# kubegems/modelx

Measured on AMD Instinct MI355X. Metric: push+pull GiB/s end-to-end (S3->HBM, digest-verified), 1/2/4/8 MI355X, higher is better.
Workload: dtype uint8; 1 GPU; model=synthetic-8GiB-blob, global_batch=1, seq_len=0, parallelism=dp1-presigned-s3-pipelined

## Files before the change

core/src/engine.cpp:

```cpp
#include <hip/hip_runtime.h>
#include <openssl/evp.h>
#include <pybind11/pybind11.h>
#include <pybind11/stl.h>

#include <atomic>
#include <chrono>
#include <condition_variable>
#include <cstring>
#include <deque>
#include <map>
#include <memory>
#include <mutex>
#include <queue>
#include <stdexcept>
#include <string_view>
#include <thread>
#include <unordered_set>
#include <vector>

#include "modelx/device_abi.hpp"
#include "modelx/http.hpp"
#include "modelx/tar_host.hpp"
#include "modelx/zstd_core.hpp"
#include "modelx/zstd_host.hpp"

namespace py = pybind11;
using namespace modelx;
using modelx::abi::ChunkLeavesDesc;
using modelx::abi::CopySeg;
using modelx::abi::kDedupMaxProbes;
using modelx::abi::PackSeg;
using modelx::abi::TarEntry;
using zstdhost::SeekEntry;

static uint32_t zstd_flags() {
  static uint32_t f = [] {
    const char* v = getenv("MODELX_ZSTD_FLAGS");
    return v ? (uint32_t)atoi(v) : 0u;
  }();
  return f;
}

#define HIP_CHECK(expr)                                                                 \
  do {                                                                                  \
    hipError_t _e = (expr);                                                             \
    if (_e != hipSuccess)                                                               \
      throw std::runtime_error(std::string("HIP error: ") + hipGetErrorString(_e) +     \
                               " at " #expr);                                           \
  } while (0)

namespace {

double now_s() {
  return std::chrono::duration<double>(std::chrono::steady_clock::now().time_since_epoch())
      .count();
}

uint64_t expected_leaf_count(uint64_t size, uint64_t chunk_size) {
  return size ? (size - 1) / chunk_size + 1 : 1;
}

uint32_t checked_leaf_count(const char* who, size_t leaves_bytes, uint64_t chunk_size,
                            uint64_t size) {
  if (chunk_size == 0) throw std::runtime_error(std::string(who) + ": chunk_size is 0");
  if (leaves_bytes % 32)
    throw std::runtime_error(std::string(who) + ": leaves length " +
                             std::to_string(leaves_bytes) + " is not a multiple of 32");
  uint64_t want = expected_leaf_count(size, chunk_size);
  if (leaves_bytes / 32 != want || want > UINT32_MAX)
    throw std::runtime_error(std::string(who) + ": " + std::to_string(leaves_bytes / 32) +
                             " leaves for " + std::to_string(size) + " bytes at chunk size " +
                             std::to_string(chunk_size) + " (expected " +
                             std::to_string(want) + ")");
  return static_cast<uint32_t>(want);
}

struct Slot {
  char* host = nullptr;
  hipEvent_t event = nullptr;
  size_t bytes = 0;
};

struct Range {
  uint64_t offset;
  uint64_t length;
};

class DeviceBuffer {
 public:
  DeviceBuffer() = default;
  explicit DeviceBuffer(size_t bytes) { HIP_CHECK(hipMalloc(&p_, bytes)); }
  DeviceBuffer(DeviceBuffer&& o) noexcept : p_(o.p_) { o.p_ = nullptr; }
  DeviceBuffer& operator=(DeviceBuffer&& o) noexcept {
    std::swap(p_, o.p_);
    return *this;
  }
  ~DeviceBuffer() {
    if (p_) hipFree(p_);
  }
  template <class T = void>
  T* get() const { return static_cast<T*>(p_); }
  explicit operator bool() const { return p_ != nullptr; }

 private:
  void* p_ = nullptr;
};

class DeviceScratch {
 public:
  template <class T = void>
  T* reserve(size_t bytes) {
    if (cap_ < bytes) {
      cap_ = 0;
      buf_ = DeviceBuffer();
      buf_ = DeviceBuffer(bytes);
      cap_ = bytes;
    }
    return buf_.get<T>();
  }

 private:
  DeviceBuffer buf_;
  size_t cap_ = 0;
};

class ConnPool {
 public:
  std::unique_ptr<http::ClientConn> checkout(const std::string& host, int port, bool tls) {
    std::lock_guard<std::mutex> lk(mu_);
    auto& v = pool_[(tls ? "https:" : "http:") + host + ":" + std::to_string(port)];
    if (!v.empty()) {
      auto c = std::move(v.back());
      v.pop_back();
      return c;
    }
    return std::make_unique<http::ClientConn>(host, port, tls);
  }
  void checkin(std::unique_ptr<http::ClientConn> c) {
    if (!c || !c->connected()) return;
    std::lock_guard<std::mutex> lk(mu_);
    auto& v = pool_[(c->tls() ? "https:" : "http:") + c->host() + ":" +
                    std::to_string(c->port())];
    if (v.size() < 64) v.push_back(std::move(c));
  }

 private:
  std::mutex mu_;
  std::map<std::string, std::vector<std::unique_ptr<http::ClientConn>>> pool_;
};

class GpuEngine {
 public:
  GpuEngine(int device, int num_slots, size_t slot_bytes, int num_streams)
      : device_(device), slot_bytes_(slot_bytes) {
    HIP_CHECK(hipSetDevice(device_));
    slots_.resize(num_slots);
    for (auto& s : slots_) {
      HIP_CHECK(hipHostMalloc(reinterpret_cast<void**>(&s.host), slot_bytes,
                              hipHostMallocDefault));
      HIP_CHECK(hipEventCreateWithFlags(&s.event, hipEventDisableTiming));
      free_.push(&s);
    }
    streams_.resize(num_streams);
    for (auto& st : streams_) HIP_CHECK(hipStreamCreateWithFlags(&st, hipStreamNonBlocking));
    HIP_CHECK(hipStreamCreateWithFlags(&hash_stream_, hipStreamNonBlocking));
    HIP_CHECK(hipEventCreateWithFlags(&zs_staged_, hipEventDisableTiming));
  }

  ~GpuEngine() {
    for (auto& st : streams_) hipStreamDestroy(st);
    hipStreamDestroy(hash_stream_);
    hipEventDestroy(zs_staged_);
    for (auto& s : slots_) {
      if (s.event) hipEventDestroy(s.event);
      if (s.host) hipHostFree(s.host);
    }
  }


  py::dict pull_to_device(const std::string& url,
                          const std::map<std::string, std::string>& headers, uint64_t size,
                          uintptr_t dst_ptr, int num_conns, uint64_t base_offset = 0) {
    std::string leaves;
    return pull_impl(url, headers, size, dst_ptr, num_conns, base_offset, 0, &leaves, nullptr);
  }

  py::dict pull_ranges_to_device(const std::string& url,
                                 const std::map<std::string, std::string>& headers,
                                 const std::vector<std::pair<uint64_t, uint64_t>>& ranges,
                                 uintptr_t dst_ptr, int num_conns) {
    std::string leaves;
    std::vector<Range> rs;
    uint64_t total = 0;
    for (auto& r : ranges) {
      for (uint64_t off = 0; off < r.second; off += slot_bytes_)
        rs.push_back({r.first + off, std::min<uint64_t>(slot_bytes_, r.second - off)});
      total += r.second;
    }
    return pull_impl(url, headers, total, dst_ptr, num_conns, 0, 0, &leaves, &rs);
  }

  py::tuple pull_to_device_hashed(const std::string& url,
                                  const std::map<std::string, std::string>& headers,
                                  uint64_t size, uintptr_t dst_ptr, int num_conns,
                                  uint64_t chunk_size) {
    std::string leaves;
    py::dict stats =
        pull_impl(url, headers, size, dst_ptr, num_conns, 0, chunk_size, &leaves, nullptr);
    return py::make_tuple(stats, py::bytes(leaves));
  }

  py::dict pull_impl(const std::string& url, const std::map<std::string, std::string>& headers,
                     uint64_t size, uintptr_t dst_ptr, int num_conns, uint64_t base_offset,
                     uint64_t hash_chunk, std::string* leaves_out,
                     const std::vector<Range>* explicit_ranges) {
    DeviceBuffer dleaves;
    uint32_t total_chunks = 0;
    if (hash_chunk) {
      if (slot_bytes_ % hash_chunk != 0)
        throw std::runtime_error("slot_bytes must be a multiple of chunk_size");
      total_chunks = size ? static_cast<uint32_t>((size + hash_chunk - 1) / hash_chunk) : 1;
      dleaves = DeviceBuffer(static_cast<size_t>(total_chunks) * 32);
    }
    py::gil_scoped_release release;
    HIP_CHECK(hipSetDevice(device_));
    double t0 = now_s();

    constexpr uint64_t kSlotsPerRequest = 4;
    std::vector<Range> ranges;
    if (explicit_ranges) {
      ranges = *explicit_ranges;
    } else {
      uint64_t super = slot_bytes_ * kSlotsPerRequest;
      for (uint64_t off = 0; off < size; off += super)
        ranges.push_back({off, std::min<uint64_t>(super, size - off)});
    }
    std::atomic<size_t> next_range{0};
    std::mutex err_mu;
    std::string error;
    std::atomic<uint64_t> net_bytes{0};
    std::atomic<long> net_ns{0};

    std::atomic<bool> done_submitting{false};
    std::thread reclaimer([&] {
      while (true) {
        Slot* s = nullptr;
        {
          std::unique_lock<std::mutex> lk(mu_);
          cv_pending_.wait(lk, [&] {
            return !pending_.empty() || (done_submitting.load() && pending_.empty());
          });
          if (pending_.empty()) break;
          s = pending_.front();
          pending_.pop_front();
        }
        hipEventSynchronize(s->event);
        {
          std::lock_guard<std::mutex> lk(mu_);
          free_.push(s);
        }
        cv_free_.notify_all();
      }
    });

    http::Url u = http::Url::parse(url);
    std::vector<std::thread> workers;
    std::atomic<int> stream_rr{0};
    for (int w = 0; w < num_conns; w++) {
      workers.emplace_back([&, w] {
        if (hipError_t e = hipSetDevice(device_); e != hipSuccess) {
          std::lock_guard<std::mutex> lk(err_mu);
          if (error.empty()) error = std::string("hip: ") + hipGetErrorString(e);
          return;
        }
        auto conn_holder = conn_pool_.checkout(u.host, u.port, u.scheme == "https");
        http::ClientConn& conn = *conn_holder;
        http::Headers h;
        for (auto& kv : headers) h[kv.first] = kv.second;
        while (true) {
          Range r;
          {
            size_t i = next_range.fetch_add(1);
            if (i >= ranges.size()) break;
            {
              std::lock_guard<std::mutex> lk(err_mu);
              if (!error.empty()) break;
            }
            r = ranges[i];
          }
          bool ok = false;
          for (int attempt = 0; attempt < 3 && !ok; attempt++) {
            double tn = now_s();
            if (!begin_range_fetch(conn, u, h, {r.offset + base_offset, r.length})) continue;
            ok = true;
            for (uint64_t poff = 0; poff < r.length && ok; poff += slot_bytes_) {
              uint64_t plen = std::min<uint64_t>(slot_bytes_, r.length - poff);
              Slot* slot = acquire_slot();
              if (!conn.read_body_exact(slot->host, plen)) {
                conn.close_fd();
                release_slot(slot);
                ok = false;
                break;
              }
              uint64_t abs_off = r.offset + poff;
              hipStream_t st = streams_[stream_rr.fetch_add(1) % streams_.size()];
              hipError_t e = hipMemcpyAsync(reinterpret_cast<char*>(dst_ptr) + abs_off,
                                            slot->host, plen, hipMemcpyHostToDevice, st);
              if (e == hipSuccess && hash_chunk) {
                uint32_t first_chunk = static_cast<uint32_t>(abs_off / hash_chunk);
                uint32_t n_chunks =
                    static_cast<uint32_t>((plen + hash_chunk - 1) / hash_chunk);
                e = modelx_sha256_chunk_leaves(
                    reinterpret_cast<char*>(dst_ptr) + abs_off, plen, hash_chunk,
                    dleaves.get<char>() + static_cast<size_t>(first_chunk) * 32,
                    n_chunks, st);
              }
              if (e == hipSuccess) e = hipEventRecord(slot->event, st);
              if (e != hipSuccess) {
                {
                  std::lock_guard<std::mutex> lk(err_mu);
                  if (error.empty()) error = std::string("hip: ") + hipGetErrorString(e);
                }
                release_slot(slot);
                ok = false;
                attempt = 3;
                break;
              }
              {
                std::lock_guard<std::mutex> lk(mu_);
                pending_.push_back(slot);
              }
              cv_pending_.notify_all();
            }
            if (ok) {
              net_ns.fetch_add(static_cast<long>((now_s() - tn) * 1e9));
              net_bytes.fetch_add(r.length);
            }
          }
          if (!ok) {
            std::lock_guard<std::mutex> lk(err_mu);
            if (error.empty()) error = "range fetch failed @" + std::to_string(r.offset);
            break;
          }
        }
        conn_pool_.checkin(std::move(conn_holder));
      });
    }
    for (auto& t : workers) t.join();
    done_submitting.store(true);
    cv_pending_.notify_all();
    reclaimer.join();
    for (auto& st : streams_) HIP_CHECK(hipStreamSynchronize(st));
    if (hash_chunk) {
      leaves_out->resize(static_cast<size_t>(total_chunks) * 32);
      HIP_CHECK(hipMemcpy(&(*leaves_out)[0], dleaves.get(), leaves_out->size(),
                          hipMemcpyDeviceToHost));
      dleaves = DeviceBuffer();
    }
    double t1 = now_s();
    {
      std::lock_guard<std::mutex> lk(err_mu);
      if (!error.empty()) throw std::runtime_error("pull_to_device: " + error);
    }
    py::gil_scoped_acquire acquire;
    py::dict stats;
    stats["seconds"] = t1 - t0;
    stats["bytes"] = size;
    stats["gib_per_s"] = size / (t1 - t0) / (1 << 30);
    stats["net_conn_seconds"] = net_ns.load() / 1e9;
    return stats;
  }


  py::bytes sha256_chunk_leaves(uintptr_t dev_ptr, uint64_t size, uint64_t chunk_size) {
    if (chunk_size == 0) throw std::runtime_error("sha256_chunk_leaves: chunk_size is 0");
    HIP_CHECK(hipSetDevice(device_));
    uint32_t nchunks = static_cast<uint32_t>(expected_leaf_count(size, chunk_size));
    std::string out;
    {
      py::gil_scoped_release release;
      DeviceBuffer dleaves(static_cast<size_t>(nchunks) * 32);
      HIP_CHECK(modelx_sha256_chunk_leaves(reinterpret_cast<void*>(dev_ptr), size, chunk_size,
                                           dleaves.get(), nchunks, hash_stream_));
      out.resize(static_cast<size_t>(nchunks) * 32);
      HIP_CHECK(hipStreamSynchronize(hash_stream_));
      HIP_CHECK(hipMemcpy(&out[0], dleaves.get(), out.size(), hipMemcpyDeviceToHost));
    }
    return py::bytes(out);
  }

  py::bytes sha256_multibuf(const std::vector<std::pair<uintptr_t, uint64_t>>& bufs) {
    HIP_CHECK(hipSetDevice(device_));
    uint32_t n = static_cast<uint32_t>(bufs.size());
    if (n == 0) return py::bytes("");
    std::vector<const void*> hptrs(n);
    std::vector<uint64_t> hlens(n);
    for (uint32_t i = 0; i < n; i++) {
      hptrs[i] = reinterpret_cast<const void*>(bufs[i].first);
      hlens[i] = bufs[i].second;
    }
    std::string out;
    {
      py::gil_scoped_release release;
      DeviceBuffer dptrs(n * sizeof(void*));
      DeviceBuffer dlens(n * sizeof(uint64_t));
      DeviceBuffer ddig(static_cast<size_t>(n) * 32);
      HIP_CHECK(hipMemcpyAsync(dptrs.get(), hptrs.data(), n * sizeof(void*),
                               hipMemcpyHostToDevice, hash_stream_));
      HIP_CHECK(hipMemcpyAsync(dlens.get(), hlens.data(), n * sizeof(uint64_t),
                               hipMemcpyHostToDevice, hash_stream_));
      HIP_CHECK(modelx_sha256_multibuf(dptrs.get<const void*>(), dlens.get<uint64_t>(), n,
                                       ddig.get(), hash_stream_));
      out.resize(static_cast<size_t>(n) * 32);
      HIP_CHECK(hipStreamSynchronize(hash_stream_));
      HIP_CHECK(hipMemcpy(&out[0], ddig.get(), out.size(), hipMemcpyDeviceToHost));
    }
    return py::bytes(out);
  }

  py::bytes read_device(uintptr_t src_ptr, uint64_t size) {
    HIP_CHECK(hipSetDevice(device_));
    std::string out(size, '\0');
    {
      py::gil_scoped_release release;
      HIP_CHECK(hipMemcpy(&out[0], reinterpret_cast<void*>(src_ptr), size,
                          hipMemcpyDeviceToHost));
    }
    return py::bytes(out);
  }

  py::bytes sha256_canonical_device(uintptr_t src_ptr, uint64_t size) {
    HIP_CHECK(hipSetDevice(device_));
    unsigned char md[32];
    {
      py::gil_scoped_release release;
      std::unique_ptr<EVP_MD_CTX, decltype(&EVP_MD_CTX_free)> ctx(EVP_MD_CTX_new(),
                                                                  &EVP_MD_CTX_free);
      if (!ctx || EVP_DigestInit_ex(ctx.get(), EVP_sha256(), nullptr) != 1)
        throw std::runtime_error("EVP sha256 init failed");
      hipError_t e = drain_device(src_ptr, size, [&](const char* p, uint64_t len) {
        EVP_DigestUpdate(ctx.get(), p, len);
        return true;
      });
      if (e != hipSuccess)
        throw std::runtime_error(std::string("sha256_canonical_device: hip: ") +
                                 hipGetErrorString(e));
      unsigned int mdlen = 0;
      EVP_DigestFinal_ex(ctx.get(), md, &mdlen);
    }
    return py::bytes(reinterpret_cast<char*>(md), 32);
  }


  py::dict push_part_from_device(const std::string& url, const std::string& method,
                                 const std::map<std::string, std::string>& headers,
                                 uintptr_t src_ptr, uint64_t size) {
    py::gil_scoped_release release;
    HIP_CHECK(hipSetDevice(device_));
    double t0 = now_s();
    http::Url u = http::Url::parse(url);
    auto conn_holder = conn_pool_.checkout(u.host, u.port, u.scheme == "https");
    http::ClientConn& conn = *conn_holder;
    http::Headers h;
    for (auto& kv : headers) h[kv.first] = kv.second;
    if (!conn.send_request(method, u.target(), h, static_cast<int64_t>(size)))
      throw std::runtime_error("push: send_request failed");
    bool sent = true;
    HIP_CHECK(drain_device(src_ptr, size, [&](const char* p, uint64_t len) {
      return sent = conn.send_body(p, len);
    }));
    if (!sent) throw std::runtime_error("push: send_body failed");
    int status = 0;
    http::Headers rh;
    if (!conn.read_response_head(&status, &rh)) throw std::runtime_error("push: no response");
    char drain[4096];
    while (conn.read_body(drain, sizeof drain) > 0) {
    }
    conn_pool_.checkin(std::move(conn_holder));
    double t1 = now_s();
    if (status < 200 || status >= 300)
      throw std::runtime_error("push: HTTP " + std::to_string(status));
    py::gil_scoped_acquire acquire;
    py::dict stats;
    stats["seconds"] = t1 - t0;
    stats["bytes"] = size;
    stats["status"] = status;
    return stats;
  }


  py::list tar_index(uintptr_t tar_ptr, uint64_t tar_len) {
    HIP_CHECK(hipSetDevice(device_));
    uint32_t max_entries = tarhost::kMaxIndexEntries;
    std::vector<TarEntry> entries;
    uint32_t count = 0, error = 0;
    {
      py::gil_scoped_release release;
      DeviceBuffer dentries(max_entries * sizeof(TarEntry));
      DeviceBuffer dcount_buf(2 * sizeof(uint32_t));
      uint32_t* dcount = dcount_buf.get<uint32_t>();
      HIP_CHECK(modelx_tar_index(reinterpret_cast<void*>(tar_ptr), tar_len,
                                 dentries.get<TarEntry>(), max_entries, dcount, dcount + 1,
                                 hash_stream_));
      HIP_CHECK(hipStreamSynchronize(hash_stream_));
      HIP_CHECK(hipMemcpy(&count, dcount, sizeof count, hipMemcpyDeviceToHost));
      HIP_CHECK(hipMemcpy(&error, dcount + 1, sizeof error, hipMemcpyDeviceToHost));
// ... 341 lines not shown
                    reinterpret_cast<uint8_t*>(dleaves + off[i] * 32), size, cs,
                    (uint32_t)off[i], 0};
      }
      ChunkLeavesDesc* ddescs = zs_descs_.reserve<ChunkLeavesDesc>(n * sizeof(ChunkLeavesDesc));
      HIP_CHECK(hipMemcpyAsync(ddescs, descs.data(), n * sizeof(ChunkLeavesDesc),
                               hipMemcpyHostToDevice, hash_stream_));
      HIP_CHECK(modelx_sha256_chunk_leaves_many(ddescs, (uint32_t)n, (uint32_t)total,
                                                hash_stream_));
      HIP_CHECK(hipStreamSynchronize(hash_stream_));
      host.resize(total * 32);
      HIP_CHECK(hipMemcpy(&host[0], dleaves, host.size(), hipMemcpyDeviceToHost));
    }
    for (size_t i = 0; i < n; i++)
      res.emplace_back(host.data() + off[i] * 32, (size_t)nchunks[i] * 32);
    return res;
  }

  static uint64_t zstd_compress_bound(uint64_t size, uint32_t frame_raw) {
    using namespace modelx::zstd;
    if (frame_raw == 0) frame_raw = 128 << 10;
    uint64_t nframes = size ? (size + frame_raw - 1) / frame_raw : 1;
    uint64_t stride = (uint64_t)frame_raw + 64 + 3 * ((frame_raw + kBlockMax - 1) / kBlockMax);
    return nframes * stride + 8 + nframes * 8 + 9;
  }


  void dedup_reset(uint64_t cap_pow2) {
    if (cap_pow2 && ((cap_pow2 & (cap_pow2 - 1)) || cap_pow2 < kDedupMaxProbes))
      throw std::runtime_error("dedup_reset: capacity " + std::to_string(cap_pow2) +
                               " is not a power of two >= " +
                               std::to_string(kDedupMaxProbes));
    HIP_CHECK(hipSetDevice(device_));
    py::gil_scoped_release release;
    std::lock_guard<std::mutex> lk(dedup_mu_);
    if (cap_pow2 == 0) cap_pow2 = dedup_cap_ ? dedup_cap_ : (1ull << 22);
    if (dedup_cap_ != cap_pow2) {
      dedup_cap_ = 0;
      dedup_table_ = DeviceBuffer();
      dedup_table_ = DeviceBuffer(cap_pow2 * 48);
      dedup_cap_ = cap_pow2;
    }
    if (!dedup_dropped_) dedup_dropped_ = DeviceBuffer(sizeof(uint32_t));
    HIP_CHECK(hipMemsetAsync(dedup_table_.get(), 0, dedup_cap_ * 48, hash_stream_));
    HIP_CHECK(hipMemsetAsync(dedup_dropped_.get(), 0, sizeof(uint32_t), hash_stream_));
    HIP_CHECK(hipStreamSynchronize(hash_stream_));
  }

  uint32_t dedup_register(py::bytes leaves, uintptr_t base, uint64_t chunk_size,
                          uint64_t total) {
    std::string lv = leaves;
    uint32_t nleaves = checked_leaf_count("dedup_register", lv.size(), chunk_size, total);
    HIP_CHECK(hipSetDevice(device_));
    py::gil_scoped_release release;
    std::string uniq;
    std::vector<uint32_t> idx;
    {
      std::unordered_set<std::string_view> seen;
      seen.reserve(nleaves);
      idx.reserve(nleaves);
      for (uint32_t i = 0; i < nleaves; i++)
        if (seen.insert(std::string_view(lv.data() + (size_t)i * 32, 32)).second)
          idx.push_back(i);
      uniq.reserve(idx.size() * 36);
      for (uint32_t i : idx) uniq.append(lv.data() + (size_t)i * 32, 32);
      uniq.append(reinterpret_cast<const char*>(idx.data()), idx.size() * 4);
    }
    uint32_t n = static_cast<uint32_t>(idx.size());
    std::lock_guard<std::mutex> lk(dedup_mu_);
    if (!dedup_table_) {
      uint64_t cap = 1ull << 22;
      dedup_table_ = DeviceBuffer(cap * 48);
      HIP_CHECK(hipMemsetAsync(dedup_table_.get(), 0, cap * 48, hash_stream_));
      dedup_cap_ = cap;
      dedup_dropped_ = DeviceBuffer(sizeof(uint32_t));
      HIP_CHECK(hipMemsetAsync(dedup_dropped_.get(), 0, sizeof(uint32_t), hash_stream_));
    }
    char* dleaves = ds_leaves_.reserve<char>(uniq.size());
    HIP_CHECK(hipMemcpyAsync(dleaves, uniq.data(), uniq.size(), hipMemcpyHostToDevice,
                             hash_stream_));
    const uint32_t* didx = reinterpret_cast<const uint32_t*>(dleaves + (size_t)n * 32);
    HIP_CHECK(modelx_dedup_insert(dleaves, didx, n, base, chunk_size, total,
                                  dedup_table_.get(), dedup_cap_,
                                  dedup_dropped_.get<uint32_t>(), hash_stream_));
    uint32_t dropped = 0;
    HIP_CHECK(hipStreamSynchronize(hash_stream_));
    HIP_CHECK(hipMemcpy(&dropped, dedup_dropped_.get(), sizeof dropped, hipMemcpyDeviceToHost));
    return dropped;
  }

  py::tuple dedup_pull(py::bytes expect, uintptr_t dst_ptr, uint64_t chunk_size,
                       uint64_t total) {
    std::string lv = expect;
    uint32_t n = checked_leaf_count("dedup_pull", lv.size(), chunk_size, total);
    std::vector<std::pair<uint64_t, uint64_t>> missing;
    uint64_t deduped = 0;
    if (total && dedup_table_) {
      HIP_CHECK(hipSetDevice(device_));
      py::gil_scoped_release release;
      std::lock_guard<std::mutex> lk(dedup_mu_);
      void* dleaves = ds_leaves_.reserve(lv.size());
      uint64_t* daddr = ds_addr_.reserve<uint64_t>((uint64_t)n * 8);
      uint64_t* dlen = ds_len_.reserve<uint64_t>((uint64_t)n * 8);
      HIP_CHECK(hipMemcpyAsync(dleaves, lv.data(), lv.size(), hipMemcpyHostToDevice,
                               hash_stream_));
      HIP_CHECK(modelx_dedup_probe(dleaves, n, chunk_size, total, dedup_table_.get(),
                                   dedup_cap_, daddr, dlen, hash_stream_));
      HIP_CHECK(modelx_dedup_gather(daddr, dlen, n, dst_ptr, chunk_size, hash_stream_));
      std::vector<uint64_t> haddr(n);
      HIP_CHECK(hipStreamSynchronize(hash_stream_));
      HIP_CHECK(hipMemcpy(haddr.data(), daddr, (uint64_t)n * 8, hipMemcpyDeviceToHost));
      for (uint32_t i = 0; i < n; i++) {
        uint64_t off = (uint64_t)i * chunk_size;
        uint64_t ln = total - off < chunk_size ? total - off : chunk_size;
        if (haddr[i] != 0) {
          deduped += ln;
        } else if (!missing.empty() && missing.back().first + missing.back().second == off) {
          missing.back().second += ln;
        } else {
          missing.emplace_back(off, ln);
        }
      }
    } else {
      if (total) missing.emplace_back(0, total);
    }
    py::list out;
    for (auto& m : missing) out.append(py::make_tuple(m.first, m.second));
    return py::make_tuple(out, deduped);
  }

  void synchronize() {
    HIP_CHECK(hipSetDevice(device_));
    for (auto& st : streams_) HIP_CHECK(hipStreamSynchronize(st));
    HIP_CHECK(hipStreamSynchronize(hash_stream_));
  }

 private:
  Slot* acquire_slot() {
    std::unique_lock<std::mutex> lk(mu_);
    cv_free_.wait(lk, [&] { return !free_.empty(); });
    Slot* s = free_.front();
    free_.pop();
    return s;
  }
  void release_slot(Slot* s) {
    {
      std::lock_guard<std::mutex> lk(mu_);
      free_.push(s);
    }
    cv_free_.notify_all();
  }

  class SlotLease {
   public:
    explicit SlotLease(GpuEngine& eng) : eng_(eng) {
      std::unique_lock<std::mutex> lk(eng_.mu_);
      eng_.cv_free_.wait(lk, [&] { return eng_.free_.size() >= 2; });
      for (Slot*& s : slot_) {
        s = eng_.free_.front();
        eng_.free_.pop();
      }
    }
    SlotLease(const SlotLease&) = delete;
    ~SlotLease() {
      for (int i = 0; i < 2; i++)
        if (in_flight_[i]) (void)hipEventSynchronize(slot_[i]->event);
      {
        std::lock_guard<std::mutex> lk(eng_.mu_);
        for (Slot* s : slot_) eng_.free_.push(s);
      }
      eng_.cv_free_.notify_all();
    }
    const char* host(int i) const { return slot_[i]->host; }
    hipError_t fill(int i, const char* src, uint64_t len, hipStream_t st) {
      hipError_t e = hipMemcpyAsync(slot_[i]->host, src, len, hipMemcpyDeviceToHost, st);
      if (e == hipSuccess) e = hipEventRecord(slot_[i]->event, st);
      if (e == hipSuccess) in_flight_[i] = true;
      return e;
    }
    hipError_t wait(int i) {
      in_flight_[i] = false;
      return hipEventSynchronize(slot_[i]->event);
    }

   private:
    GpuEngine& eng_;
    Slot* slot_[2];
    bool in_flight_[2] = {false, false};
  };

  template <class Consume>
  hipError_t drain_device(uintptr_t src_ptr, uint64_t size, Consume&& consume) {
    if (!size) return hipSuccess;
    const char* src = reinterpret_cast<const char*>(src_ptr);
    hipStream_t st_a = streams_[push_rr_.fetch_add(1) % streams_.size()];
    hipStream_t st_b = streams_[push_rr_.fetch_add(1) % streams_.size()];
    SlotLease lease(*this);
    int cur = 0, nxt = 1;
    uint64_t off = 0;
    uint64_t cur_len = std::min<uint64_t>(slot_bytes_, size);
    hipError_t e = lease.fill(cur, src, cur_len, st_a);
    while (e == hipSuccess && off < size) {
      uint64_t next_off = off + cur_len;
      uint64_t next_len = next_off < size ? std::min<uint64_t>(slot_bytes_, size - next_off) : 0;
      if (next_len) {
        e = lease.fill(nxt, src + next_off, next_len, st_b);
        if (e != hipSuccess) break;
        std::swap(st_a, st_b);
      }
      e = lease.wait(cur);
      if (e != hipSuccess || !consume(lease.host(cur), cur_len)) break;
      std::swap(cur, nxt);
      off = next_off;
      cur_len = next_len;
    }
    return e;
  }

  bool begin_range_fetch(http::ClientConn& conn, const http::Url& u, http::Headers h,
                         const Range& r) {
    h["Range"] =
        "bytes=" + std::to_string(r.offset) + "-" + std::to_string(r.offset + r.length - 1);
    if (!conn.send_request("GET", u.target(), h, -1)) return false;
    int status = 0;
    http::Headers rh;
    if (!conn.read_response_head(&status, &rh)) return false;
    auto cl = rh.find("Content-Length");
    if (status != 206 || cl == rh.end() ||
        atoll(cl->second.c_str()) != static_cast<long long>(r.length)) {
      conn.close_fd();
      return false;
    }
    return true;
  }

  int device_;
  size_t slot_bytes_;
  std::atomic<int> push_rr_{0};
  std::vector<Slot> slots_;
  std::queue<Slot*> free_;
  std::deque<Slot*> pending_;
  std::vector<hipStream_t> streams_;
  hipStream_t hash_stream_ = nullptr;
  std::mutex mu_;
  std::condition_variable cv_free_, cv_pending_;
  ConnPool conn_pool_;
  std::mutex zstd_mu_;
  DeviceScratch zs_compress_, zs_seqs_, zs_sizes_, zs_segs_;
  DeviceScratch zs_frames_, zs_lit_, zs_rc_;
  hipEvent_t zs_staged_ = nullptr;
  DeviceScratch zs_leaves_, zs_descs_;
  std::mutex dedup_mu_;
  DeviceBuffer dedup_table_;
  uint64_t dedup_cap_ = 0;
  DeviceBuffer dedup_dropped_;
  DeviceScratch ds_leaves_, ds_addr_, ds_len_;
};

bool hip_available() {
  int n = 0;
  return hipGetDeviceCount(&n) == hipSuccess && n > 0;
}

int hip_device_count() {
  int n = 0;
  if (hipGetDeviceCount(&n) != hipSuccess) return 0;
  return n;
}

}

PYBIND11_MODULE(_core, m) {
  m.doc() = "modelx_amd native core: pinned-ring S3<->HBM engine + CDNA4 SHA-256 kernels";
  m.def("hip_available", &hip_available);
  m.def("hip_device_count", &hip_device_count);
  m.def("hip_pci_bus_id", [](int device) {
    char buf[64] = {};
    if (hipDeviceGetPCIBusId(buf, sizeof buf, device) != hipSuccess)
      throw std::runtime_error("hipDeviceGetPCIBusId failed");
    return std::string(buf);
  });

  py::class_<GpuEngine>(m, "GpuEngine")
      .def(py::init<int, int, size_t, int>(), py::arg("device") = 0, py::arg("num_slots") = 8,
           py::arg("slot_bytes") = (size_t)(64 << 20), py::arg("num_streams") = 4)
      .def("pull_to_device", &GpuEngine::pull_to_device, py::arg("url"), py::arg("headers"),
           py::arg("size"), py::arg("dst_ptr"), py::arg("num_conns") = 8,
           py::arg("base_offset") = 0)
      .def("pull_ranges_to_device", &GpuEngine::pull_ranges_to_device, py::arg("url"),
           py::arg("headers"), py::arg("ranges"), py::arg("dst_ptr"), py::arg("num_conns") = 8)
      .def("pull_to_device_hashed", &GpuEngine::pull_to_device_hashed, py::arg("url"),
           py::arg("headers"), py::arg("size"), py::arg("dst_ptr"), py::arg("num_conns") = 8,
           py::arg("chunk_size") = (uint64_t)(128 << 10))
      .def("sha256_chunk_leaves", &GpuEngine::sha256_chunk_leaves, py::arg("dev_ptr"),
           py::arg("size"), py::arg("chunk_size"))
      .def("sha256_multibuf", &GpuEngine::sha256_multibuf, py::arg("buffers"))
      .def("sha256_canonical_device", &GpuEngine::sha256_canonical_device,
           py::arg("src_ptr"), py::arg("size"))
      .def("read_device", &GpuEngine::read_device, py::arg("src_ptr"), py::arg("size"))
      .def("push_part_from_device", &GpuEngine::push_part_from_device, py::arg("url"),
           py::arg("method"), py::arg("headers"), py::arg("src_ptr"), py::arg("size"))
      .def("tar_index", &GpuEngine::tar_index, py::arg("tar_ptr"), py::arg("tar_len"))
      .def("tar_scatter", &GpuEngine::tar_scatter, py::arg("tar_ptr"), py::arg("segs"))
      .def("tar_pack", &GpuEngine::tar_pack, py::arg("dst_ptr"), py::arg("dst_cap"),
           py::arg("members"))
      .def("dedup_reset", &GpuEngine::dedup_reset, py::arg("cap_pow2") = (uint64_t)0)
      .def("dedup_register", &GpuEngine::dedup_register, py::arg("leaves"), py::arg("base"),
           py::arg("chunk_size"), py::arg("total"))
      .def("dedup_pull", &GpuEngine::dedup_pull, py::arg("expect"), py::arg("dst_ptr"),
           py::arg("chunk_size"), py::arg("total"))
      .def("zstd_decompress_many", &GpuEngine::zstd_decompress_many, py::arg("items"))
      .def("sha256_chunk_leaves_many", &GpuEngine::sha256_chunk_leaves_many,
           py::arg("items"))
      .def("zstd_compress_device", &GpuEngine::zstd_compress_device, py::arg("src_ptr"),
           py::arg("size"), py::arg("frame_raw"), py::arg("dst_ptr"), py::arg("dst_cap"))
      .def("zstd_decompress_device", &GpuEngine::zstd_decompress_device, py::arg("src_ptr"),
           py::arg("src_len"), py::arg("dst_ptr"), py::arg("dst_cap"))
      .def("synchronize", &GpuEngine::synchronize);

  m.def(
      "tar_pack_layout",
      [](const std::vector<std::pair<std::string, uint64_t>>& members) {
        tarhost::PackLayout lay = tarhost::pack_layout(members);
        py::list entries;
        for (auto& e : lay.entries) {
          py::dict d;
          d["header_off"] = e.header_off;
          d["header_len"] = e.header_len;
          d["payload_off"] = e.payload_off;
          d["size"] = e.size;
          entries.append(std::move(d));
        }
        py::dict out;
        out["headers"] = py::bytes(lay.headers);
        out["entries"] = entries;
        out["total"] = lay.total;
        return out;
      },
      py::arg("members"));
  m.def("zstd_compress_bound", &GpuEngine::zstd_compress_bound, py::arg("size"),
        py::arg("frame_raw") = (uint32_t)(128 << 10));
  m.def(
      "zstd_compress_cpu",
      [](py::bytes data, uint32_t frame_raw) {
        std::string s = data;
        std::vector<uint8_t> out;
        {
          py::gil_scoped_release release;
          out = zstdhost::compress_seekable(reinterpret_cast<const uint8_t*>(s.data()),
                                            s.size(), frame_raw);
        }
        return py::bytes(reinterpret_cast<const char*>(out.data()), out.size());
      },
      py::arg("data"), py::arg("frame_raw") = (uint32_t)(128 << 10));
  m.def("http_get", [](const std::string& url,
                       const std::map<std::string, std::string>& headers) {
    http::Url u = http::Url::parse(url);
    http::ClientConn conn(u.host, u.port, u.scheme == "https");
    http::Headers h;
    for (auto& kv : headers) h[kv.first] = kv.second;
    h["Host"] = u.host + ":" + std::to_string(u.port);
    http::ClientResponse resp;
    if (!conn.do_request("GET", u.target(), h, "", &resp))
      throw std::runtime_error("http_get: request failed (connect/TLS/socket)");
    return py::make_tuple(resp.status, py::bytes(resp.body));
  }, py::arg("url"), py::arg("headers") = std::map<std::string, std::string>{});

  m.def("sha256_host", [](py::bytes data) {
    std::string s = data;
    unsigned char md[32];
    unsigned int mdlen = 0;
    EVP_MD_CTX* ctx = EVP_MD_CTX_new();
    if (!ctx || EVP_DigestInit_ex(ctx, EVP_sha256(), nullptr) != 1) {
      if (ctx) EVP_MD_CTX_free(ctx);
      throw std::runtime_error("EVP sha256 init failed");
    }
    EVP_DigestUpdate(ctx, s.data(), s.size());
    EVP_DigestFinal_ex(ctx, md, &mdlen);
    EVP_MD_CTX_free(ctx);
    return py::bytes(reinterpret_cast<char*>(md), 32);
  });
  m.def("zstd_decompress_cpu", [](py::bytes data) {
    std::string s = data;
    std::vector<uint8_t> out;
    {
      py::gil_scoped_release release;
      out = zstdhost::decompress(reinterpret_cast<const uint8_t*>(s.data()), s.size());
    }
    return py::bytes(reinterpret_cast<const char*>(out.data()), out.size());
  });
  m.def("zstd_content_size", [](py::bytes data) {
// ... 27 lines not shown
```

modelx_amd/client/gpu.py:

```python
from __future__ import annotations

from datetime import datetime, timezone
from typing import Dict, List, Optional, Tuple

from ..wire import digest as dg
from ..wire import errors as er
from ..wire import types
from .registry import RegistryClient

DEFAULT_SLOT_BYTES = 64 << 20
DEFAULT_NUM_SLOTS = 16
DEFAULT_NUM_CONNS = 16
DEFAULT_PART_BYTES = 256 << 20
DEFAULT_PUSH_PARALLEL = 6
DEFAULT_GPU_CHUNK = 128 << 10


def _core():
    try:
        from modelx_amd import _core as core
    except ImportError as e:
        raise er.ModelxError(
            er.ErrCode.INTERNAL,
            "modelx_amd._core native extension not built "
# ... 223 lines not shown
        import time

        import torch

        comp = self.pull_blob_to_device(repository, desc, verify=verify,
                                        plan_entry=plan_entry)
        raw_size = int(desc.annotations.get(types.ANNOTATION_RAW_SIZE, 0) or 0)
        if not raw_size:
            raise er.ModelxError(er.ErrCode.UNSUPPORTED,
                                 f"+zstd blob {desc.name} lacks the raw-size annotation")
        out = torch.empty(max(raw_size, 1), dtype=torch.uint8, device=f"cuda:{self.device}")
        t0 = time.monotonic()
        try:
            got = self.engine.zstd_decompress_device(comp.data_ptr(), desc.size,
                                                     out.data_ptr(), out.numel())
        except RuntimeError as e:
            import os as _os
            import sys

            dump_dir = _os.environ.get("MODELX_ZSTD_DUMP", "")
            if dump_dir:
                try:
                    _os.makedirs(dump_dir, exist_ok=True)
                    path = _os.path.join(
                        dump_dir,
                        f"zstd_decode_fail_{desc.digest.split(':')[-1][:12]}.zst")
                    with open(path, "wb") as f:
                        f.write(bytes(comp[: desc.size].cpu().numpy().tobytes()))
                    print(f"modelx: zstd decode failed ({e}); dumped {path}; retrying once",
                          file=sys.stderr)
                except Exception:
                    pass
            else:
                print(f"modelx: zstd decode failed ({e}); retrying once "
                      "(set MODELX_ZSTD_DUMP=<dir> to keep the blob)", file=sys.stderr)
            got = self.engine.zstd_decompress_device(comp.data_ptr(), desc.size,
                                                     out.data_ptr(), out.numel())
        self.last_stats.append({"phase": "pull-zstd-decompress", "bytes": got,
                                "seconds": time.monotonic() - t0})
        if raw_size and got != raw_size:
            raise er.ModelxError(er.ErrCode.DIGEST_INVALID,
                                 f"zstd size mismatch for {desc.name}: {got} != {raw_size}")
        out = out[:got]
        raw_digest = desc.annotations.get(types.ANNOTATION_RAW_DIGEST, "")
        if verify and raw_digest:
            cs = dg.algo_chunk_size(raw_digest.split(":", 1)[0]) or DEFAULT_GPU_CHUNK
            leaves = self.engine.sha256_chunk_leaves(out.data_ptr(), got, cs)
            root = dg.root_from_leaf_bytes(leaves, cs, got)
            if root != raw_digest:
                raise er.ModelxError(er.ErrCode.DIGEST_INVALID,
                                     f"uncompressed digest mismatch for {desc.name}")
        return out

    def pull_blob_to_device(self, repository: str, desc: types.Descriptor,
                            tensor=None, verify: bool = True,
                            resume: bool = False, plan_entry=None) -> "torch.Tensor":
        import time

        import torch

        had_tensor = tensor is not None
        if tensor is None:
            tensor = torch.empty(desc.size, dtype=torch.uint8, device=f"cuda:{self.device}")
        assert tensor.numel() >= desc.size
        planned = self._plan_url(plan_entry)
        located = planned if planned else self._download_url(repository, desc)
        if located is None:
            for attempt in range(2):
                self._stream_via_registry(repository, desc, tensor)
                if not verify:
                    return tensor
                try:
                    self._verify_device_digest(tensor.data_ptr(), desc.size, desc)
                    return tensor
                except er.ModelxError:
                    if attempt:
                        raise
            return tensor
        url, headers = located

        cs = _annotated_chunk_size(desc) or (
            dg.algo_chunk_size(desc.digest.split(":", 1)[0]) or DEFAULT_GPU_CHUNK)

        def expected_leaves():
            lv = (self._plan_leaves(plan_entry, desc)
                  or self._expected_leaves(repository, desc))
            return lv if lv is not None and leaves_usable(lv, desc.size, cs) else None

        if resume and had_tensor:
            expect = expected_leaves()
            if expect is not None:
                got = self.engine.sha256_chunk_leaves(tensor.data_ptr(), desc.size, cs)
                ranges = self._bad_chunk_ranges(got, expect, cs, desc.size)
                fetched = self._fetch_ranges(url, headers, tensor.data_ptr(), ranges)
                self.last_stats.append({"phase": "pull-resume", "bytes": fetched,
                                        "skipped": desc.size - fetched})
                if verify:
                    self._verify_device_digest(tensor.data_ptr(), desc.size, desc)
                return tensor

        if self.dedup and self._dedup_registered:
            expect = expected_leaves()
            if expect is not None:
                t0 = time.monotonic()
                missing, dedup_bytes = self.engine.dedup_pull(
                    expect, tensor.data_ptr(), cs, desc.size)
                if dedup_bytes:
                    fetched = self._fetch_ranges(url, headers, tensor.data_ptr(), missing)
                    stats = {"phase": "pull-dedup", "bytes": fetched,
                             "dedup_bytes": dedup_bytes,
                             "seconds": time.monotonic() - t0}
                    self.last_stats.append(stats)
                    if verify:
                        got = self.engine.sha256_chunk_leaves(tensor.data_ptr(),
                                                              desc.size, cs)
                        bad = self._bad_chunk_ranges(got, expect, cs, desc.size)
                        if bad:
                            import sys

                            fetched_offs = set()
                            for off, ln in missing:
                                for o in range(off, off + ln, cs):
                                    fetched_offs.add(o)
                            kinds = {"gathered": 0, "fetched": 0}
                            for off, ln in bad:
                                for o in range(off, off + ln, cs):
                                    kinds["fetched" if o in fetched_offs else "gathered"] += 1
                            print(f"modelx: dedup refetch {desc.name}: "
                                  f"{len(bad)} ranges, chunks by origin {kinds}",
                                  file=sys.stderr)
                            stats["refetched_bytes"] = self._fetch_ranges(
                                url, headers, tensor.data_ptr(), bad)
                            stats["refetched_ranges"] = len(bad)
                            got = self.engine.sha256_chunk_leaves(tensor.data_ptr(),
                                                                  desc.size, cs)
                        root = dg.root_from_leaf_bytes(got, cs, desc.size)
                        target = desc.annotations.get(types.ANNOTATION_CHUNK_DIGEST, "")
                        if dg.algo_chunk_size(desc.digest.split(":", 1)[0] if desc.digest
                                              else ""):
                            target = desc.digest
                        if target and root != target:
                            raise er.ModelxError(
                                er.ErrCode.DIGEST_INVALID,
                                f"GPU chunk digest mismatch for {desc.name}: {root}")
                    self.register_chunks(tensor, expect, cs, desc.size)
                    return tensor

        expect_digest = ""
        algo_cs = dg.algo_chunk_size(desc.digest.split(":", 1)[0]) if desc.digest else None
        if algo_cs:
            expect_digest = desc.digest
        elif desc.annotations.get(types.ANNOTATION_CHUNK_DIGEST, ""):
            expect_digest = desc.annotations[types.ANNOTATION_CHUNK_DIGEST]
        stream_hash = (verify and expect_digest
                       and self.slot_bytes % cs == 0 and desc.size > 0)
        t0 = time.monotonic()
        if stream_hash:
            stats, leaves = self.engine.pull_to_device_hashed(
                url, headers, desc.size, tensor.data_ptr(), self.num_conns, cs)
            stats["name"] = desc.name
            stats["phase"] = "pull-transfer-hashed"
            self.last_stats.append(stats)
            got = dg.root_from_leaf_bytes(leaves, cs, desc.size)
            if got == expect_digest:
                self.last_stats.append({"phase": "pull-verify", "bytes": desc.size,
                                        "seconds": time.monotonic() - t0 - stats["seconds"]})
                self.register_chunks(tensor, leaves, cs, desc.size)
                return tensor
        else:
            stats = self.engine.pull_to_device(url, headers, desc.size, tensor.data_ptr(),
                                               self.num_conns)
            stats["name"] = desc.name
            stats["phase"] = "pull-transfer"
            self.last_stats.append(stats)
        if not verify:
            return tensor
        t0 = time.monotonic()
        try:
            self._verify_device_digest(tensor.data_ptr(), desc.size, desc)
        except er.ModelxError as first_err:
            expect = expected_leaves()
            if expect is None:
                raise er.ModelxError(
                    er.ErrCode.DIGEST_INVALID,
                    f"{first_err.message} [size={desc.size} media={desc.media_type} "
                    f"path=no-leaves-sidecar]") from first_err
            got = self.engine.sha256_chunk_leaves(tensor.data_ptr(), desc.size, cs)
            ranges = self._bad_chunk_ranges(got, expect, cs, desc.size)
            if not ranges:
                raise er.ModelxError(
                    er.ErrCode.DIGEST_INVALID,
                    f"{first_err.message} [size={desc.size} media={desc.media_type} "
                    f"path=leaves-match-but-root-differs]") from first_err
            self._fetch_ranges(url, headers, tensor.data_ptr(), ranges)
            self.last_stats.append({"phase": "pull-chunk-refetch",
                                    "bytes": sum(r[1] for r in ranges)})
            try:
                self._verify_device_digest(tensor.data_ptr(), desc.size, desc)
            except er.ModelxError as second_err:
                raise er.ModelxError(
                    er.ErrCode.DIGEST_INVALID,
                    f"{second_err.message} [size={desc.size} media={desc.media_type} "
                    f"path=refetch-did-not-fix ranges={len(ranges)}]") from second_err
        self.last_stats.append({"phase": "pull-verify", "bytes": desc.size,
                                "seconds": time.monotonic() - t0})
        return tensor

    def _pull_zstd_batched(self, repository: str, jobs, verify: bool,
                           parallel: int) -> Dict[object, "torch.Tensor"]:
        import time

        import torch

        wave_cap = self.ZSTD_WAVE_CAP
        if len(jobs) > 1:
            total_raw = sum(int(d.annotations.get(types.ANNOTATION_RAW_SIZE, 0) or 0)
                            for _, d, _ in jobs)
            if total_raw > wave_cap:
                out: Dict[object, "torch.Tensor"] = {}
                wave, acc = [], 0
                for job in jobs:
                    raw = int(job[1].annotations.get(types.ANNOTATION_RAW_SIZE, 0) or 0)
                    if wave and acc + raw > wave_cap:
                        out.update(self._pull_zstd_batched(repository, wave, verify,
                                                           parallel))
                        wave, acc = [], 0
                    wave.append(job)
                    acc += raw
                if wave:
                    out.update(self._pull_zstd_batched(repository, wave, verify,
                                                       parallel))
                return out

        def one(job):
            key, desc, entry = job
            return key, self.pull_blob_to_device(repository, desc, verify=verify,
                                                 plan_entry=entry)

        if parallel > 1 and len(jobs) > 1:
            from concurrent.futures import ThreadPoolExecutor

            with ThreadPoolExecutor(max_workers=parallel) as ex:
                comp = dict(ex.map(one, jobs))
        else:
            comp = dict(one(j) for j in jobs)
        outs: Dict[object, "torch.Tensor"] = {}
        items = []
        metas = []
        for key, desc, _ in jobs:
            raw_size = int(desc.annotations.get(types.ANNOTATION_RAW_SIZE, 0) or 0)
            if not raw_size:
                raise er.ModelxError(er.ErrCode.UNSUPPORTED,
                                     f"+zstd blob {desc.name} lacks the raw-size annotation")
            o = torch.empty(max(raw_size, 1), dtype=torch.uint8,
                            device=f"cuda:{self.device}")
            items.append((comp[key].data_ptr(), desc.size, o.data_ptr(), o.numel()))
            outs[key] = o
            metas.append((key, desc, raw_size))
        t0 = time.monotonic()
        sizes = self.engine.zstd_decompress_many(items)
        self.last_stats.append({"phase": "pull-zstd-decompress-batched",
                                "bytes": sum(sizes), "blobs": len(items),
                                "seconds": time.monotonic() - t0})
        for (key, desc, raw_size), got in zip(metas, sizes):
            if got != raw_size:
                raise er.ModelxError(er.ErrCode.DIGEST_INVALID,
                                     f"zstd size mismatch for {desc.name}: "
                                     f"{got} != {raw_size}")
            outs[key] = outs[key][:got]
        if verify:
            vitems, vmeta = [], []
            for key, desc, raw_size in metas:
                rd = desc.annotations.get(types.ANNOTATION_RAW_DIGEST, "")
                if not rd:
                    continue
                cs = dg.algo_chunk_size(rd.split(":", 1)[0]) or DEFAULT_GPU_CHUNK
                o = outs[key]
                vitems.append((o.data_ptr(), o.numel(), cs))
                vmeta.append((desc, cs, o.numel(), rd))
            if vitems:
                t0 = time.monotonic()
                leaves_list = self.engine.sha256_chunk_leaves_many(vitems)
                for (desc, cs, sz, rd), leaves in zip(vmeta, leaves_list):
                    if dg.root_from_leaf_bytes(leaves, cs, sz) != rd:
                        raise er.ModelxError(
                            er.ErrCode.DIGEST_INVALID,
                            f"uncompressed digest mismatch for {desc.name}")
                self.last_stats.append({"phase": "pull-zstd-raw-verify-batched",
                                        "bytes": sum(v[1] for v in vitems),
                                        "seconds": time.monotonic() - t0})
        return outs

    def pull_to_gpu(self, repository: str, version: str = "",
                    verify: bool = True, parallel: int = 1,
                    expand_dirs: bool = False) -> Dict[str, "torch.Tensor"]:
        plan = self.remote.get_pull_plan(repository, version)
        if plan and plan.get("manifest"):
            manifest = types.Manifest.from_dict(plan["manifest"])
            plan_blobs = plan.get("blobs") or {}
        else:
            manifest = self.remote.get_manifest(repository, version)
            plan_blobs = {}
        descs = [d for d in manifest.blobs
                 if d.size and d.media_type != types.MEDIA_TYPE_MODEL_LEAVES]
        zstd_descs = [d for d in descs
                      if d.media_type == types.MEDIA_TYPE_MODEL_FILE_ZSTD]
        plain_descs = [d for d in descs
                       if d.media_type != types.MEDIA_TYPE_MODEL_FILE_ZSTD]
# ... 501 lines not shown
```

Measured before the change: 23.64 GiB/s.

## Defer pull chunk hashing to one post-transfer pass; split push slots into halves

```diff
diff --git a/core/src/engine.cpp b/core/src/engine.cpp
--- a/core/src/engine.cpp
+++ b/core/src/engine.cpp
@@ -77,7 +77,7 @@
 
 struct Slot {
   char* host = nullptr;
-  hipEvent_t event = nullptr;
+  hipEvent_t event[2] = {nullptr, nullptr};
   size_t bytes = 0;
 };
 
@@ -152,13 +152,22 @@
 class GpuEngine {
  public:
   GpuEngine(int device, int num_slots, size_t slot_bytes, int num_streams)
-      : device_(device), slot_bytes_(slot_bytes) {
+      : device_(device),
+        slot_bytes_(slot_bytes),
+        half_bytes_((slot_bytes / 2) & ~size_t{15}) {
+    if (half_bytes_ == 0)
+      throw std::runtime_error("GpuEngine: slot_bytes " + std::to_string(slot_bytes) +
+                               " is too small: a slot must hold two halves of at least "
+                               "16 bytes (slot_bytes >= 32)");
+    if (num_slots < 1 || num_streams < 1)
+      throw std::runtime_error("GpuEngine: num_slots and num_streams must be at least 1");
     HIP_CHECK(hipSetDevice(device_));
     slots_.resize(num_slots);
     for (auto& s : slots_) {
       HIP_CHECK(hipHostMalloc(reinterpret_cast<void**>(&s.host), slot_bytes,
                               hipHostMallocDefault));
-      HIP_CHECK(hipEventCreateWithFlags(&s.event, hipEventDisableTiming));
+      for (hipEvent_t& ev : s.event)
+        HIP_CHECK(hipEventCreateWithFlags(&ev, hipEventDisableTiming));
       free_.push(&s);
     }
     streams_.resize(num_streams);
@@ -172,7 +181,8 @@
     hipStreamDestroy(hash_stream_);
     hipEventDestroy(zs_staged_);
     for (auto& s : slots_) {
-      if (s.event) hipEventDestroy(s.event);
+      for (hipEvent_t ev : s.event)
+        if (ev) hipEventDestroy(ev);
       if (s.host) hipHostFree(s.host);
     }
   }
@@ -217,9 +227,11 @@
     DeviceBuffer dleaves;
     uint32_t total_chunks = 0;
     if (hash_chunk) {
-      if (slot_bytes_ % hash_chunk != 0)
-        throw std::runtime_error("slot_bytes must be a multiple of chunk_size");
-      total_chunks = size ? static_cast<uint32_t>((size + hash_chunk - 1) / hash_chunk) : 1;
+      uint64_t want = expected_leaf_count(size, hash_chunk);
+      if (want > UINT32_MAX)
+        throw std::runtime_error("pull_to_device_hashed: " + std::to_string(want) +
+                                 " chunks exceed the kernel's 32-bit chunk index");
+      total_chunks = static_cast<uint32_t>(want);
       dleaves = DeviceBuffer(static_cast<size_t>(total_chunks) * 32);
     }
     py::gil_scoped_release release;
@@ -254,7 +266,7 @@
           s = pending_.front();
           pending_.pop_front();
         }
-        hipEventSynchronize(s->event);
+        hipEventSynchronize(s->event[0]);
         {
           std::lock_guard<std::mutex> lk(mu_);
           free_.push(s);
@@ -306,16 +318,7 @@
               hipStream_t st = streams_[stream_rr.fetch_add(1) % streams_.size()];
               hipError_t e = hipMemcpyAsync(reinterpret_cast<char*>(dst_ptr) + abs_off,
                                             slot->host, plen, hipMemcpyHostToDevice, st);
-              if (e == hipSuccess && hash_chunk) {
-                uint32_t first_chunk = static_cast<uint32_t>(abs_off / hash_chunk);
-                uint32_t n_chunks =
-                    static_cast<uint32_t>((plen + hash_chunk - 1) / hash_chunk);
-                e = modelx_sha256_chunk_leaves(
-                    reinterpret_cast<char*>(dst_ptr) + abs_off, plen, hash_chunk,
-                    dleaves.get<char>() + static_cast<size_t>(first_chunk) * 32,
-                    n_chunks, st);
-              }
-              if (e == hipSuccess) e = hipEventRecord(slot->event, st);
+              if (e == hipSuccess) e = hipEventRecord(slot->event[0], st);
               if (e != hipSuccess) {
                 {
                   std::lock_guard<std::mutex> lk(err_mu);
@@ -351,7 +354,11 @@
     cv_pending_.notify_all();
     reclaimer.join();
     for (auto& st : streams_) HIP_CHECK(hipStreamSynchronize(st));
-    if (hash_chunk) {
+    if (hash_chunk && error.empty()) {
+      hipStream_t hst = streams_[hash_rr_.fetch_add(1) % streams_.size()];
+      HIP_CHECK(modelx_sha256_chunk_leaves(reinterpret_cast<void*>(dst_ptr), size, hash_chunk,
+                                           dleaves.get(), total_chunks, hst));
+      HIP_CHECK(hipStreamSynchronize(hst));
       leaves_out->resize(static_cast<size_t>(total_chunks) * 32);
       HIP_CHECK(hipMemcpy(&(*leaves_out)[0], dleaves.get(), leaves_out->size(),
                           hipMemcpyDeviceToHost));
@@ -999,39 +1006,29 @@
 
   class SlotLease {
    public:
-    explicit SlotLease(GpuEngine& eng) : eng_(eng) {
-      std::unique_lock<std::mutex> lk(eng_.mu_);
-      eng_.cv_free_.wait(lk, [&] { return eng_.free_.size() >= 2; });
-      for (Slot*& s : slot_) {
-        s = eng_.free_.front();
-        eng_.free_.pop();
-      }
-    }
+    explicit SlotLease(GpuEngine& eng) : eng_(eng), slot_(eng.acquire_slot()) {}
     SlotLease(const SlotLease&) = delete;
     ~SlotLease() {
       for (int i = 0; i < 2; i++)
-        if (in_flight_[i]) (void)hipEventSynchronize(slot_[i]->event);
-      {
-        std::lock_guard<std::mutex> lk(eng_.mu_);
-        for (Slot* s : slot_) eng_.free_.push(s);
-      }
-      eng_.cv_free_.notify_all();
-    }
-    const char* host(int i) const { return slot_[i]->host; }
+        if (in_flight_[i]) (void)hipEventSynchronize(slot_->event[i]);
+      eng_.release_slot(slot_);
+    }
+    const char* host(int i) const { return slot_->host + i * eng_.half_bytes_; }
     hipError_t fill(int i, const char* src, uint64_t len, hipStream_t st) {
-      hipError_t e = hipMemcpyAsync(slot_[i]->host, src, len, hipMemcpyDeviceToHost, st);
-      if (e == hipSuccess) e = hipEventRecord(slot_[i]->event, st);
+      hipError_t e = hipMemcpyAsync(slot_->host + i * eng_.half_bytes_, src, len,
+                                    hipMemcpyDeviceToHost, st);
+      if (e == hipSuccess) e = hipEventRecord(slot_->event[i], st);
       if (e == hipSuccess) in_flight_[i] = true;
       return e;
     }
     hipError_t wait(int i) {
       in_flight_[i] = false;
-      return hipEventSynchronize(slot_[i]->event);
+      return hipEventSynchronize(slot_->event[i]);
     }
 
    private:
     GpuEngine& eng_;
-    Slot* slot_[2];
+    Slot* slot_;
     bool in_flight_[2] = {false, false};
   };
 
@@ -1044,11 +1041,11 @@
     SlotLease lease(*this);
     int cur = 0, nxt = 1;
     uint64_t off = 0;
-    uint64_t cur_len = std::min<uint64_t>(slot_bytes_, size);
+    uint64_t cur_len = std::min<uint64_t>(half_bytes_, size);
     hipError_t e = lease.fill(cur, src, cur_len, st_a);
     while (e == hipSuccess && off < size) {
       uint64_t next_off = off + cur_len;
-      uint64_t next_len = next_off < size ? std::min<uint64_t>(slot_bytes_, size - next_off) : 0;
+      uint64_t next_len = next_off < size ? std::min<uint64_t>(half_bytes_, size - next_off) : 0;
       if (next_len) {
         e = lease.fill(nxt, src + next_off, next_len, st_b);
         if (e != hipSuccess) break;
@@ -1082,7 +1079,9 @@
 
   int device_;
   size_t slot_bytes_;
+  size_t half_bytes_;
   std::atomic<int> push_rr_{0};
+  std::atomic<unsigned> hash_rr_{0};
   std::vector<Slot> slots_;
   std::queue<Slot*> free_;
   std::deque<Slot*> pending_;
diff --git a/modelx_amd/client/gpu.py b/modelx_amd/client/gpu.py
--- a/modelx_amd/client/gpu.py
+++ b/modelx_amd/client/gpu.py
@@ -399,8 +399,7 @@
             expect_digest = desc.digest
         elif desc.annotations.get(types.ANNOTATION_CHUNK_DIGEST, ""):
             expect_digest = desc.annotations[types.ANNOTATION_CHUNK_DIGEST]
-        stream_hash = (verify and expect_digest
-                       and self.slot_bytes % cs == 0 and desc.size > 0)
+        stream_hash = verify and expect_digest and desc.size > 0
         t0 = time.monotonic()
         if stream_hash:
             stats, leaves = self.engine.pull_to_device_hashed(
```

New measurement: 24.48 GiB/s, median of 5. 3.5% higher.
